# fbreitwieser/krakenuniq

Measured on AMD Instinct MI355X. Metric: Mreads/s (150 bp), higher is better.
Workload: dtype u64

## Files before the change

### krakenuniq_amd/csrc/ku_short.hip

```cpp
#include <cstdlib>
#include <type_traits>

#include "ku_device.h"

#define KS_WAVES 4
#ifndef KS_KCT_LOG2
#define KS_KCT_LOG2 8
#endif
#define KS_FLOOR_EVERY 64u
#define KS_HQ 64
#define KS_PAD 16
#ifdef KU_ABLATION
#define KS_ABL(bit) ((ablate & (bit)) != 0)
#else
#define KS_ABL(bit) false
#endif

template <int ITEMS> struct KsGeom {
  static constexpr int MAXN = 64 * ITEMS;
  static constexpr int NWORDS = (MAXN + 31 + 15) / 16 + 3;
  static constexpr int NCODES = (MAXN + 64) / 16 + 4;
  static constexpr int NAMB = (NWORDS + 1) / 2 + 2;
  static constexpr int NMM = MAXN + 64 + 32;
  static constexpr int TCAP_LOG2 = ITEMS <= 2 ? 8 : (ITEMS <= 4 ? 9 : 10);
  static constexpr int KCT_LOG2 = KS_KCT_LOG2;
  static constexpr int RCT_LOG2 = 6;
};

template <int ITEMS, bool WIN, bool SCAN, bool HQ> struct KsWaveLds {
  using G = KsGeom<ITEMS>;
  static constexpr int TCAP = 1 << G::TCAP_LOG2;
  std::conditional_t<HQ, uint2, uint32_t> hq[HQ ? KS_HQ : 0];
  uint32_t codes[SCAN ? G::NCODES : 0];
  uint32_t amb[SCAN ? G::NAMB : 0];
  uint32_t mm[SCAN ? G::NMM : 0];
  uint32_t tkey[TCAP];
  uint32_t tcnt[TCAP];
  uint32_t kk[SCAN ? 1 << G::KCT_LOG2 : 0], kc[SCAN ? 1 << G::KCT_LOG2 : 0];
  uint32_t rk[1 << G::RCT_LOG2], rc[1 << G::RCT_LOG2];
  uint32_t misc[4];
  uint16_t tlist[WIN ? TCAP : G::MAXN];
};

struct __attribute__((packed, aligned(4))) KsQuad {
  uint32_t x, y, z, w;
};
__device__ __forceinline__ uint64_t ks_quad_key(const KsQuad &q) { return ((uint64_t)q.y << 32) | q.x; }
__device__ __forceinline__ uint4 ks_quad_header(const KsQuad &q) { return make_uint4(q.x, q.y, q.z, q.w); }

__device__ __forceinline__ bool ks_less64(uint64_t a, uint64_t b) { return (int64_t)(a - b) < 0; }

__device__ __forceinline__ void ks_wave_sync() {
  __builtin_amdgcn_fence(__ATOMIC_RELEASE, "wavefront");
  __builtin_amdgcn_wave_barrier();
  __builtin_amdgcn_fence(__ATOMIC_ACQUIRE, "wavefront");
}

template <int LOG2>
__device__ __forceinline__ void ks_ct_flush(uint32_t *key, uint32_t *cnt, uint32_t *used, unsigned long long *global,
                                            uint32_t lane, uint32_t *hot = nullptr) {
  ks_wave_sync();
  for (uint32_t i = lane; i < (1u << LOG2); i += 64) {
    uint32_t kk = key[i];
#ifdef KS_DIAG_NOHOT
    if (kk == 1) kk = 0;
#endif
    if (hot && kk == 1) { *hot = cnt[i]; kk = 0; }
    if (kk) atomicAdd(&global[kk - 1], (unsigned long long)cnt[i]);
    key[i] = 0;
    cnt[i] = 0;
  }
  if (lane == 0) *used = 0;
  ks_wave_sync();
}

__device__ __forceinline__ uint32_t ks_bmin4(uint32_t a, uint32_t b) {
  const uint32_t m = ((((a | 0x80808080u) - b) & 0x80808080u) >> 7) * 0xFFu;
  return (b & m) | (a & ~m);
}

#define KS_RCT_SLOT 0x40000000u
__device__ __forceinline__ uint32_t ks_rct_node(uint32_t id, const KuTaxDev &tax) {
  return (id & KS_RCT_SLOT) ? ((id & ~KS_RCT_SLOT) ? tax.slot_node[id & ~KS_RCT_SLOT] : 0u) : id;
}
template <int LOG2>
__device__ __forceinline__ void ks_rct_add(uint32_t *key, uint32_t *cnt, uint32_t *used, uint32_t id, const KuTaxDev &tax,
                                           unsigned long long *global) {
  uint32_t h = (id * 2654435761u) >> (32 - LOG2);
#pragma unroll 1
  for (int probe = 0; probe < 8; ++probe) {
    uint32_t cur = key[h];
    if (cur == 0) { key[h] = id + 1; *used += 1; cur = id + 1; }
    if (cur == id + 1) { cnt[h] += 1; return; }
    h = (h + 1) & ((1u << LOG2) - 1);
  }
  atomicAdd(&global[ks_rct_node(id, tax)], 1ull);
}
template <int LOG2>
__device__ __forceinline__ void ks_rct_flush(uint32_t *key, uint32_t *cnt, uint32_t *used, const KuTaxDev &tax,
                                             unsigned long long *global, uint32_t lane, uint32_t *hot = nullptr) {
  ks_wave_sync();
  for (uint32_t i = lane; i < (1u << LOG2); i += 64) {
    uint32_t kk = key[i];
#ifdef KS_DIAG_NOHOT
    if (kk - 1 == KS_RCT_SLOT) kk = 0;
#endif
    if (hot && kk - 1 == KS_RCT_SLOT) { *hot = cnt[i]; kk = 0; }
    if (kk) atomicAdd(&global[ks_rct_node(kk - 1, tax)], (unsigned long long)cnt[i]);
    key[i] = 0;
    cnt[i] = 0;
  }
  if (lane == 0) *used = 0;
  ks_wave_sync();
}

template <int LOG2, bool TRACK>
__device__ __forceinline__ void ks_tab_add(uint32_t *t_key, uint32_t *t_cnt, uint32_t *n_distinct, uint32_t slot, uint32_t count) {
  uint32_t h = (slot * 2654435761u) >> (32 - LOG2);
  for (;;) {
    uint32_t cur = __hip_atomic_load(&t_key[h], __ATOMIC_RELAXED, __HIP_MEMORY_SCOPE_WORKGROUP);
    if (cur == 0) {
      uint32_t old = atomicCAS(&t_key[h], 0u, slot + 1);
      if (TRACK && old == 0) atomicAdd(n_distinct, 1u);
      cur = old == 0 ? slot + 1 : old;
    }
    if (cur == slot + 1) {
      atomicAdd(&t_cnt[h], count);
      break;
    }
    h = (h + 1) & ((1u << LOG2) - 1);
  }
}

template <int LOG2>
__device__ __forceinline__ uint32_t ks_tab_resolve(uint32_t *t_key, uint32_t *t_cnt, uint16_t *t_list, uint32_t *list_len,
                                                   const KuTaxDev &tax, uint32_t lane, uint32_t *urow = nullptr) {
  constexpr uint32_t TCAP = 1u << LOG2;
  if (lane == 0) *list_len = 0;
  ks_wave_sync();
  for (uint32_t i = lane; i < TCAP; i += 64)
    if (t_key[i]) t_list[atomicAdd(list_len, 1u)] = (uint16_t)i;
  ks_wave_sync();
  const uint32_t n_list = *list_len;
  uint32_t my_max = 0;
  for (uint32_t e = lane; e < n_list; e += 64) {
    const uint32_t pos = t_list[e];
    const uint32_t sl = t_key[pos] - 1;
    if (urow) atomicAdd(&urow[sl], t_cnt[pos] & 0xffffu);
    uint32_t score = 0;
    for (uint32_t i = tax.slot_anc_off[sl], i_end = tax.slot_anc_off[sl + 1]; i < i_end; ++i) {
      const uint32_t s = tax.slot_anc[i];
      uint32_t h = (s * 2654435761u) >> (32 - LOG2);
      for (;;) {
        const uint32_t cur = t_key[h];
        if (cur == s + 1) { score += t_cnt[h] & 0xffffu; break; }
        if (cur == 0) break;
        h = (h + 1) & (TCAP - 1);
      }
    }
    atomicAdd(&t_cnt[pos], score << 16);
    my_max = max(my_max, score);
  }
  my_max = ku_wave_max_u32(my_max);
  ks_wave_sync();
  uint32_t last = 0, res = 0;
  bool firstt = true;
  for (;;) {
    uint32_t my_min = 0xFFFFFFFFu;
    for (uint32_t e = lane; e < n_list; e += 64) {
      const uint32_t pos = t_list[e];
      const uint32_t s = t_key[pos] - 1;
      if ((t_cnt[pos] >> 16) == my_max && s > last) my_min = min(my_min, s);
    }
    my_min = ku_wave_min_u32(my_min);
    if (my_min == 0xFFFFFFFFu) break;
    const uint32_t node = tax.slot_node[my_min];
    res = firstt ? node : ku_lca_nodes(tax.node_parent, res, node);
    firstt = false;
    last = my_min;
  }
  ks_wave_sync();
  for (uint32_t e = lane; e < n_list; e += 64) {
    const uint32_t pos = t_list[e];
    t_key[pos] = 0;
    t_cnt[pos] = 0;
  }
  ks_wave_sync();
  return res;
}

__device__ __forceinline__ uint32_t ks_gload(const uint32_t *p) {
  return __hip_atomic_load(p, __ATOMIC_RELAXED, __HIP_MEMORY_SCOPE_AGENT);
}
__device__ __noinline__ void ks_floor_scan(const uint8_t *registers, uint32_t *hll_floor, uint32_t rs, uint32_t lane) {
  const uint4 *row = reinterpret_cast<const uint4 *>(registers + (size_t)rs * KU_HLL_M) + 4 * lane;
  const uint32_t cur = ks_gload(&hll_floor[rs]);
  uint32_t lo = 0x7f7f7f7fu;
#pragma unroll
  for (int q = 0; q < 4; ++q) {
    const uint4 x = row[q];
    lo = ks_bmin4(lo, ks_bmin4(ks_bmin4(x.x, x.y), ks_bmin4(x.z, x.w)));
  }
  lo = min(min(lo & 0xffu, (lo >> 8) & 0xffu), min((lo >> 16) & 0xffu, lo >> 24));
  lo = ku_wave_min_u32(lo);
  if (lane == 0 && lo > cur) atomicMax(&hll_floor[rs], lo);
}

__device__ __noinline__ void ks_hq_drain(const uint2 *q, uint32_t fill, uint8_t *registers, uint32_t lane) {
  ks_wave_sync();
  if (lane < fill) {
    const uint2 e = q[lane];
    uint8_t *r = registers + (size_t)e.x * KU_HLL_M + (e.y & (KU_HLL_M - 1u));
    ku_hll_raise(r, (uint32_t)*r, e.y >> KU_HLL_P);
  }
  ks_wave_sync();
}

__device__ __noinline__ void ks_spill_add(uint32_t *g_key, uint32_t *g_cnt, uint32_t mask, uint32_t slot, uint32_t count) {
  uint32_t h = (slot * 2654435761u) & mask;
  for (;;) {
    uint32_t cur = ks_gload(&g_key[h]);
    if (cur == 0) {
      uint32_t old = atomicCAS(&g_key[h], 0u, slot + 1);
      cur = old == 0 ? slot + 1 : old;
    }
    if (cur == slot + 1) {
      atomicAdd(&g_cnt[h], count);
      break;
    }
    h = (h + 1) & mask;
  }
}
__device__ __noinline__ void ks_spill_migrate(uint32_t *t_key, uint32_t *t_cnt, uint32_t tcap, uint32_t *g_key, uint32_t *g_cnt,
                                              uint32_t mask, bool wipe, uint32_t lane) {
  if (wipe) {
    for (uint32_t i = lane; i <= mask; i += 64) { g_key[i] = 0; g_cnt[i] = 0; }
    __threadfence();
  }
  ks_wave_sync();
  for (uint32_t i = lane; i < tcap; i += 64) {
    const uint32_t kk = t_key[i];
    if (kk) {
      ks_spill_add(g_key, g_cnt, mask, kk - 1, t_cnt[i] & 0xffffu);
      t_key[i] = 0;
      t_cnt[i] = 0;
    }
  }
  ks_wave_sync();
}
__device__ __noinline__ uint32_t ks_spill_resolve(uint32_t *g_key, uint32_t *g_cnt, uint32_t mask, const uint32_t *slot_anc_off,
                                                  const uint32_t *slot_anc, const uint32_t *slot_node, const uint32_t *node_parent,
                                                  uint32_t lane) {
  __threadfence();
  uint32_t my_max = 0;
  for (uint32_t pos = lane; pos <= mask; pos += 64) {
    const uint32_t kk = ks_gload(&g_key[pos]);
    if (!kk) continue;
    uint32_t score = 0;
    for (uint32_t i = slot_anc_off[kk - 1], i_end = slot_anc_off[kk]; i < i_end; ++i) {
      const uint32_t s = slot_anc[i];
      uint32_t h = (s * 2654435761u) & mask;
      for (;;) {
        const uint32_t cur = ks_gload(&g_key[h]);
        if (cur == s + 1) { score += ks_gload(&g_cnt[h]) & 0xffffu; break; }
        if (cur == 0) break;
        h = (h + 1) & mask;
      }
    }
    atomicAdd(&g_cnt[pos], score << 16);
    my_max = max(my_max, score);
  }
  my_max = ku_wave_max_u32(my_max);
  __threadfence();
  uint32_t last = 0, res = 0;
  bool firstt = true;
  for (;;) {
    uint32_t my_min = 0xFFFFFFFFu;
    for (uint32_t pos = lane; pos <= mask; pos += 64) {
      const uint32_t kk = ks_gload(&g_key[pos]);
      if (kk && (ks_gload(&g_cnt[pos]) >> 16) == my_max && kk - 1 > last) my_min = min(my_min, kk - 1);
    }
    my_min = ku_wave_min_u32(my_min);
    if (my_min == 0xFFFFFFFFu) break;
    const uint32_t node = slot_node[my_min];
    res = firstt ? node : ku_lca_nodes(node_parent, res, node);
    firstt = false;
    last = my_min;
  }
  for (uint32_t pos = lane; pos <= mask; pos += 64)
    if (ks_gload(&g_key[pos])) { g_key[pos] = 0; g_cnt[pos] = 0; }
  __threadfence();
  return res;
}

template <int ITEMS>
__device__ __forceinline__ uint32_t ks_g_insert_items(unsigned long long *g_key, uint64_t g_mask, const uint32_t (&slot)[ITEMS],
                                                      const uint64_t (&hash)[ITEMS], const bool (&want)[ITEMS], uint32_t *err) {
  unsigned long long key[ITEMS], old[ITEMS];
  uint64_t h[ITEMS];
#pragma unroll
  for (int j = 0; j < ITEMS; ++j) {
    key[j] = ((unsigned long long)(slot[j] + 1) << 32) | ks_encode(hash[j]);
    h[j] = ks_mix(key[j]) & g_mask;
  }
#pragma unroll
  for (int j = 0; j < ITEMS; ++j) old[j] = want[j] ? atomicCAS(&g_key[h[j]], 0ull, key[j]) : key[j];
  uint32_t fresh_n = 0;
#pragma unroll
  for (int j = 0; j < ITEMS; ++j) {
    bool fresh = want[j] && old[j] == 0ull;
    if (want[j] && old[j] != 0ull && old[j] != key[j]) {
      bool placed = false;
      for (uint32_t probe = 1; probe < 4096 && !placed; ++probe) {
        h[j] = (h[j] + 1) & g_mask;
        const unsigned long long o = atomicCAS(&g_key[h[j]], 0ull, key[j]);
        fresh = o == 0ull;
        placed = o == 0ull || o == key[j];
      }
      if (!placed) atomicOr(err, 4u);
    }
    fresh_n += (uint32_t)__popcll(__ballot(fresh));
  }
  return fresh_n;
}

#ifndef KS_OCC2
#define KS_OCC2 6
#endif
#define KS_OCC(ITEMS) ((ITEMS) == 2 ? KS_OCC2 : 4)
template <int ITEMS, bool DO_COUNTS, int KK, int MM, bool WIN, int OUT, bool ROUTE = false>
__global__ __launch_bounds__(64 * KS_WAVES, KS_OCC(ITEMS)) void ku_classify_short_kernel(
    KuDbDev db, KuTaxDev tax, KuCountsDev cnt, const uint8_t *__restrict__ seqs, uint64_t n_bytes,
    const uint64_t *__restrict__ seq_off, const uint32_t *__restrict__ seq_len, uint64_t n_reads,
    uint32_t *__restrict__ calls, uint32_t *__restrict__ taxa, uint32_t ablate, uint32_t floor_every,
    uint32_t *__restrict__ spill, uint32_t spill_cap, KuRunsOut ro, KuSparseFast sf, KuRouteIn rin) {
  using G = KsGeom<ITEMS>;
  constexpr uint32_t TCAP = 1u << G::TCAP_LOG2;
  using Lds = KsWaveLds<ITEMS, WIN, !ROUTE, DO_COUNTS && !ROUTE>;
  __shared__ Lds s_w[KS_WAVES];

  const uint32_t lane = threadIdx.x & 63u;
  const uint32_t wv = (uint32_t)__builtin_amdgcn_readfirstlane((int)(threadIdx.x >> 6));
  Lds &sw = s_w[wv];
  uint32_t *codes = sw.codes, *amb = sw.amb, *mmv = sw.mm;
  uint32_t *t_key = sw.tkey, *t_cnt = sw.tcnt;
  uint16_t *t_list = sw.tlist;
  uint16_t *amb16 = reinterpret_cast<uint16_t *>(amb);
  uint32_t *misc = sw.misc;
  const uint32_t k = KK ? (uint32_t)KK : db.k, m = KK ? (uint32_t)MM : db.nt, w = k - m + 1;
  const uint32_t key_shift = ku_key_shift(m);
  const uint32_t *tab = reinterpret_cast<const uint32_t *>(db.table);

  for (uint32_t i = lane; i < TCAP; i += 64) { t_key[i] = 0; t_cnt[i] = 0; }
  if (!ROUTE)
    for (uint32_t i = lane; i < (1u << G::KCT_LOG2); i += 64) { sw.kk[i] = 0; sw.kc[i] = 0; }
  for (uint32_t i = lane; i < (1u << G::RCT_LOG2); i += 64) { sw.rk[i] = 0; sw.rc[i] = 0; }
  if (lane < 4) misc[lane] = 0;
  ks_wave_sync();

  const uint32_t n_waves = gridDim.x * KS_WAVES;
  uint32_t *g_key = WIN ? spill + ((uint64_t)blockIdx.x * KS_WAVES + wv) * 2ull * spill_cap : nullptr;
  uint32_t *g_cnt = WIN ? g_key + spill_cap : nullptr;
  bool spill_used = false;
  unsigned long long ch_pos = 0, ch_end = 0;
  if (OUT != 0 && ro.pre_base1) {
    ch_pos = ((unsigned long long)(ro.pre_base1 - 1u) + (unsigned long long)blockIdx.x * KS_WAVES + wv) * ro.chunk;
    ch_end = ch_pos + ro.chunk;
  }
  auto runs_room = [&](uint32_t need, uint32_t keep, unsigned long long &keep_base) {
    if (ch_pos + need <= ch_end) return;
    const uint32_t want_min = keep ? 2u * (keep + need) : need;
    const uint32_t want = want_min > ro.chunk ? want_min : ro.chunk;
    unsigned long long b = 0;
    if (lane == 0) b = atomicAdd(ro.counter, (unsigned long long)want);
    b = ((unsigned long long)(uint32_t)__builtin_amdgcn_readfirstlane((int)(uint32_t)(b >> 32)) << 32) |
        (uint32_t)__builtin_amdgcn_readfirstlane((int)(uint32_t)b);
    if (keep) {
      __threadfence();
      for (uint32_t i = lane; i < keep; i += 64) {
        if (keep_base + i < ro.cap && b + i < ro.cap) {
          const uint32_t *src = reinterpret_cast<const uint32_t *>(ro.runs + keep_base + i);
          ro.runs[b + i] = make_uint2(ks_gload(src), ks_gload(src + 1));
        }
      }
      keep_base = b;
    }
    ch_pos = b + keep;
    ch_end = b + want;
  };
  uint32_t sp_fresh = 0;
  uint32_t fl_reads =
      floor_every ? (((uint32_t)blockIdx.x * KS_WAVES + wv) * 40503u >> 8) % floor_every : 0u;
  uint32_t fl_scan = 0;
  uint32_t hq_fill = 0;
  uint2 *hq = reinterpret_cast<uint2 *>(sw.hq);
  uint32_t len_n = 0;
  uint64_t off_n = 0;
  {
    const uint64_t r0 = (uint64_t)blockIdx.x * KS_WAVES + wv;
    if (ks_less64(r0, n_reads)) { len_n = seq_len[r0]; off_n = seq_off[r0]; }
  }
  for (uint64_t r = (uint64_t)blockIdx.x * KS_WAVES + wv; ks_less64(r, n_reads); r += n_waves) {
    const uint32_t rlen = len_n;
    const uint64_t roff = off_n;
    {
      const uint64_t rn = r + n_waves;
      const bool more = ks_less64(rn, n_reads);
      len_n = more ? seq_len[rn] : 0u;
      off_n = more ? seq_off[rn] : 0ull;
    }
    const uint32_t n_all = rlen >= k ? rlen - k + 1 : 0;
    uint32_t rd_first = 0, rd_cnt = 0, win0 = 0;
    bool rd_table = false, rd_spill = false;
    uint32_t call_node = 0;
    unsigned long long run_base = 0;
    uint32_t run_n = 0, run_prev = 0;
    bool run_has_prev = false;
    do {
    const uint32_t len = WIN ? min(rlen - win0, (uint32_t)G::MAXN + k - 1) : rlen;
    const uint64_t off = roff + win0;
    const uint32_t n = len >= k ? len - k + 1 : 0;
    if (DO_COUNTS) {
      if (!ROUTE && fl_scan) {
        ks_floor_scan(cnt.registers, cnt.hll_floor, fl_scan - 1u, lane);
        fl_scan = 0;
      }
      const uint32_t fill_k = misc[0], fill_r = misc[1];
      if (!ROUTE && fill_k > (1u << G::KCT_LOG2) / 2) ks_ct_flush<G::KCT_LOG2>(sw.kk, sw.kc, &misc[0], cnt.n_kmers, lane);
      if (!WIN || win0 == 0)
        if (fill_r > (1u << G::RCT_LOG2) / 2) ks_rct_flush<G::RCT_LOG2>(sw.rk, sw.rc, &misc[1], tax, cnt.n_reads, lane);
    }
    uint32_t v[ITEMS];
    bool amb_k[ITEMS];
    uint64_t hh[ITEMS];
#pragma unroll
    for (int j = 0; j < ITEMS; ++j) { v[j] = 0; amb_k[j] = false; hh[j] = 0; }

    if (ROUTE) {
      uint32_t tk[ITEMS], kbv[ITEMS];
#pragma unroll
      for (int j = 0; j < ITEMS; ++j) {
        const uint32_t p = j * 64 + lane;
        tk[j] = p < n ? taxa[off + p] : KU_ROUTE_MISS;
      }
#pragma unroll
      for (int j = 0; j < ITEMS; ++j) {
        amb_k[j] = tk[j] == KU_AMBIG;
        kbv[j] = tk[j] < KU_ROUTE_MISS ? rin.kb[tk[j] >> 5] : 0u;
      }
#pragma unroll
      for (int j = 0; j < ITEMS; ++j) v[j] = tk[j] < KU_ROUTE_MISS ? rin.ret[(uint64_t)kbv[j] + (tk[j] & 31u)] : 0u;
    } else if (n > 0) {
      constexpr uint32_t S1_LANES = (uint32_t)((G::NWORDS * 4 + 63) / 64) * 64;
      constexpr bool S1_CLAMP = S1_LANES / 4 > (uint32_t)G::NCODES || S1_LANES / 4 > 2u * G::NAMB;
      static_assert(G::NCODES - 1 >= G::NWORDS && 2 * G::NAMB - 1 >= G::NWORDS + 1, "no dump element behind the code words");
      const bool text_inside = ks_less64(off + len + 6, n_bytes);
      const uint32_t *text = reinterpret_cast<const uint32_t *>(seqs + (off & ~3ull));
      const uint32_t text_sh = (uint32_t)off & 3u, last_dw = (len - 1u) & ~3u;
#pragma unroll
      for (uint32_t pl = lane; pl < S1_LANES; pl += 64) {
        const uint32_t b0 = 4 * pl;
        const uint32_t valid = len - min(b0, len);
        uint32_t c8 = 0, a4 = 0xFu;
        if (text_inside) {
          const uint32_t *q = text + (min(b0, last_dw) >> 2);
          ku_pack_dword(__builtin_amdgcn_alignbyte(q[1], q[0], text_sh), c8, a4);
        } else if (b0 < len) {
          const uint64_t a = off + b0;
          uint32_t d = 0;
          for (uint32_t j = 0; j < 4; ++j) d |= (a + j < n_bytes ? (uint32_t)seqs[a + j] : (uint32_t)'N') << (8 * j);
          ku_pack_dword(d, c8, a4);
        }
        if (valid < 4) a4 |= (1u << (4 - valid)) - 1u;
        const uint32_t q4 = pl & 3u;
        uint32_t word = c8 << (24 - 8 * q4), ab = a4 << (12 - 4 * q4);
        word |= ku_quad_xor1(word);
        ab |= ku_quad_xor1(ab);
        word |= ku_quad_xor2(word);
        ab |= ku_quad_xor2(ab);
        const uint32_t wi = pl >> 2;
        codes[S1_CLAMP ? min(wi, (uint32_t)G::NCODES - 1u) : wi] = word;
        amb16[(S1_CLAMP ? min(wi, 2u * G::NAMB - 1u) : wi) ^ 1u] = (uint16_t)ab;
      }
      ks_wave_sync();

      const uint32_t P = n + w - 1;
      uint64_t canon[ITEMS];
      bool is_fwd[ITEMS], ok[ITEMS];
      uint32_t pk[ITEMS + 1], wr[ITEMS + 1];
      uint32_t tacc = 0xFFFFFFFFu;
      bool tie = false;
      static_assert(G::MAXN + 30 + 63 < G::NMM - 1, "the sentinels reach the dump slot");
      mmv[P + lane] = (0x03FFFFFFu - lane) << KU_PK_KEYSHIFT;
      const bool tail_round = P > (uint32_t)ITEMS * 64u;
      pk[ITEMS] = 0;
      wr[ITEMS] = (uint32_t)G::NMM - 1u;
#pragma unroll
      for (int j = 0; j <= ITEMS; ++j) {
        if (j == ITEMS && !tail_round) break;
        const uint32_t p = j * 64 + lane;
        wr[j] = p < P ? p : (uint32_t)G::NMM - 1u;
        const uint32_t wi = p >> 4, sh = (p & 15u) * 2;
        const uint32_t c0 = codes[wi], c1 = codes[wi + 1], c2 = codes[wi + 2];
        const uint64_t x = ((((uint64_t)c0 << 32) | c1) << sh >> 32 << 32) | ((((uint64_t)c1 << 32) | c2) << sh >> 32);
        const uint32_t mm = (uint32_t)(x >> (64 - 2 * m));
        const uint32_t mrc = ku_revcomp32(mm, m);
        pk[j] = ku_pk_make((mm < mrc ? mm : mrc) ^ db.xor_mask, key_shift, mm <= mrc);
        if ((m & 1u) == 0) tie |= p < P && mm == mrc;
        mmv[wr[j]] = pk[j];
        if (j < ITEMS) {
          const uint64_t fwd = x >> (64 - 2 * k);
          const uint64_t rc = ku_revcomp64(fwd, k);
          is_fwd[j] = fwd <= rc;
          canon[j] = is_fwd[j] ? fwd : rc;
          const uint32_t ai = p >> 5, as = p & 31u;
          const uint32_t a = __funnelshift_l(amb[ai + 1], amb[ai], as);
          amb_k[j] = p < n && (a >> (32 - k)) != 0;
          ok[j] = p < n && !amb_k[j];
        }
      }
      ks_wave_sync();

      uint32_t key[ITEMS], aoff[ITEMS];
      bool plus[ITEMS];
      if (KS_ABL(64u)) {
#pragma unroll
        for (int j = 0; j < ITEMS; ++j) { key[j] = 0; aoff[j] = 0; plus[j] = true; }
      } else {
        uint32_t blk = 1;
        uint32_t tj[ITEMS + 1];
#pragma unroll
        for (int j = 0; j <= ITEMS; ++j) tj[j] = 0xFFFFFFFFu;
        auto doubling = [&](auto nr_c) {
          constexpr int NR = decltype(nr_c)::value;
#pragma unroll
          for (uint32_t sft = 0; sft < 5; ++sft) {
            const uint32_t st = 1u << sft;
            if (2 * st > w) break;
            uint32_t nb[NR];
#pragma unroll
            for (int j = 0; j < NR; ++j) nb[j] = mmv[j * 64 + lane + st] + (st << 1);
            ks_wave_sync();
#pragma unroll
            for (int j = 0; j < NR; ++j) {
              tj[j] = min(tj[j], (pk[j] ^ nb[j]) - 2u);
              pk[j] = min(pk[j], nb[j]);
              mmv[wr[j]] = pk[j];
            }
            ks_wave_sync();
            blk = 2 * st;
          }
        };
        if (tail_round) doubling(std::integral_constant<int, ITEMS + 1>{});
        else doubling(std::integral_constant<int, ITEMS>{});
        if (w > blk) {
#pragma unroll
          for (int j = 0; j < ITEMS; ++j) {
            const uint32_t nbj = mmv[j * 64 + lane + (w - blk)] + ((w - blk) << 1);
            tj[j] = min(tj[j], (pk[j] ^ nbj) - 2u);
            pk[j] = min(pk[j], nbj);
          }
        }
#pragma unroll
        for (int j = 0; j <= ITEMS; ++j) tacc = min(tacc, j * 64 + lane < P ? tj[j] : 0xFFFFFFFFu);
        tie |= tacc < (1u << KU_PK_KEYSHIFT) - 2u;
#pragma unroll
        for (int j = 0; j < ITEMS; ++j) {
          const uint32_t t = (pk[j] >> 1) & 31u;
          key[j] = pk[j] >> KU_PK_KEYSHIFT;
          aoff[j] = is_fwd[j] ? t : w - 1 - t;
          plus[j] = ((pk[j] & 1u) != 0) == is_fwd[j];
        }
        if (__any(tie)) {
          ks_wave_sync();
#pragma unroll
          for (int j = 0; j <= ITEMS; ++j) {
            const uint32_t p = j * 64 + lane;
            if (p < P) {
              const uint32_t wi = p >> 4, sh = (p & 15u) * 2;
              const uint64_t two = ((uint64_t)codes[wi] << 32) | codes[wi + 1];
              const uint32_t mm = (uint32_t)((two << sh) >> (64 - 2 * m));
              const uint32_t mrc = ku_revcomp32(mm, m);
              mmv[p] = (mm < mrc ? mm : mrc) ^ db.xor_mask;
            }
          }
          ks_wave_sync();
#pragma unroll
          for (int j = 0; j < ITEMS; ++j) {
            const uint32_t p = j * 64 + lane;
            if (ok[j]) {
              uint32_t bin;
              key[j] = ku_anchor_exact(mmv + p, w, key_shift, is_fwd[j], aoff[j], bin);
              const uint32_t q = p + (is_fwd[j] ? aoff[j] : w - 1 - aoff[j]);
              const uint32_t wi = q >> 4, sh = (q & 15u) * 2;
              const uint64_t two = ((uint64_t)codes[wi] << 32) | codes[wi + 1];
              const uint32_t mmf = (uint32_t)((two << sh) >> (64 - 2 * m));
              const uint32_t rcm = ku_revcomp32(mmf, m);
              plus[j] = is_fwd[j] ? (mmf <= rcm) : (rcm <= mmf);
            }
          }
        }
      }
      const uint32_t *lp[ITEMS];
      uint32_t cand[ITEMS];
      bool act[ITEMS], ovf[ITEMS];
#pragma unroll
      for (int j = 0; j < ITEMS; ++j) {
        const uint64_t locus = ku_locus_assemble(canon[j], key[j], aoff[j], plus[j], k, m);
        hh[j] = ku_fmix64(canon[j]);
        const uint64_t line = ku_locus_line(locus, db.n_lines);
        lp[j] = tab + (ok[j] ? line : 0) * KU_LINE_DWORDS;
        act[j] = ok[j] && !KS_ABL(1u);
        if (KS_ABL(64u)) lp[j] = tab;
      }

      uint4 h4[ITEMS];
#pragma unroll
      for (int j = 0; j < ITEMS; ++j) h4[j] = *reinterpret_cast<const uint4 *>(lp[j]);
      KsQuad q[ITEMS];
      const uint32_t *ep[ITEMS];
      bool nxt[ITEMS];
      const uint32_t *const tab_end = tab + db.n_lines * KU_LINE_DWORDS;
#pragma unroll
      for (int j = 0; j < ITEMS; ++j) {
        cand[j] = ku_tag_matches(h4[j], ku_table_tag(hh[j])) & (act[j] ? 0xFFu : 0u);
        ovf[j] = act[j] && ku_line_spilled(h4[j]);
        nxt[j] = ovf[j] && cand[j] == 0;
        const uint32_t eo = nxt[j] ? (uint32_t)KU_LINE_DWORDS : KU_LINE_ENTRY0 + 3 * (__builtin_ctz(cand[j] | 0x100u) & 7u);
        ep[j] = lp[j] + eo;
        if (ep[j] == tab_end) ep[j] = tab;
      }
#pragma unroll
      for (int j = 0; j < ITEMS; ++j) q[j] = *reinterpret_cast<const KsQuad *>(ep[j]);
      uint32_t sb[ITEMS];
      if (OUT == 2 && DO_COUNTS) {
#pragma unroll
        for (int j = 0; j < ITEMS; ++j)
          sb[j] = reinterpret_cast<const uint8_t *>(lp[j] + KU_LINE_SEEN0)[__builtin_ctz(cand[j] | 0x100u) & 7u];
      }
#pragma unroll
      for (int j = 0; j < ITEMS; ++j) {
        const bool hit = cand[j] != 0 && ks_quad_key(q[j]) == canon[j];
        v[j] = hit ? q[j].z : 0u;
        if (OUT == 2 && DO_COUNTS) {
          if (hit && !sb[j] && !KS_ABL(128u)) ku_seen_mark(lp[j], (uint32_t)__builtin_ctz(cand[j]));
        }
        cand[j] &= cand[j] - 1;
        act[j] = !hit && (cand[j] != 0 || ovf[j]);
      }
      bool any = false;
#pragma unroll
      for (int j = 0; j < ITEMS; ++j) any |= act[j];
      while (any && !KS_ABL(1024u)) {
        bool pick[ITEMS], taken = false, fresh = false, ov = false;
        const uint32_t *l = tab;
        uint32_t cm = 0;
        uint64_t hsel = 0;
        KsQuad hq = {0, 0, 0, 0};
#pragma unroll
        for (int j = 0; j < ITEMS; ++j) {
          pick[j] = act[j] && !taken;
          taken |= act[j];
          if (pick[j]) { hsel = hh[j]; l = lp[j]; cm = cand[j]; ov = ovf[j]; fresh = nxt[j]; hq = q[j]; }
        }
        const uint32_t t = ku_table_tag(hsel);
        if (fresh) {
          l += KU_LINE_DWORDS;
          if (l == tab_end) l = tab;
        }
        for (;;) {
          if (fresh) {
            cm = ku_tag_matches(ks_quad_header(hq), t);
            ov = ku_line_spilled(ks_quad_header(hq));
          }
          if (cm == 0 && !ov) break;
          fresh = cm == 0;
          if (fresh) {
            l += KU_LINE_DWORDS;
            if (l == tab_end) l = tab;
          }
          const uint32_t ei = (uint32_t)__builtin_ctz(cm | 0x100u) & 7u;
          hq = *reinterpret_cast<const KsQuad *>(fresh ? l : l + KU_LINE_ENTRY0 + 3 * ei);
          if (!fresh) {
            cm &= cm - 1;
            bool same = false;
#pragma unroll
            for (int j = 0; j < ITEMS; ++j) same |= pick[j] && ks_quad_key(hq) == canon[j];
            if (same) {
#pragma unroll
              for (int j = 0; j < ITEMS; ++j)
                if (pick[j]) v[j] = hq.z;
              if (OUT == 2 && DO_COUNTS && !KS_ABL(128u)) ku_seen_mark(l, ei);
              break;
            }
          }
        }
        any = false;
#pragma unroll
        for (int j = 0; j < ITEMS; ++j) {
          if (pick[j]) act[j] = false;
          any |= act[j];
        }
      }

    }

    bool uni = false;
    uint32_t uni_slot = 0;
    uint32_t hit_first = 0;
    if (!KS_ABL(32u)) {
      uint32_t mine = 0;
#pragma unroll
      for (int j = 0; j < ITEMS; ++j)
        if (mine == 0) mine = v[j];
      const unsigned long long bal = __ballot(mine != 0);
      const uint32_t first = bal ? ku_wave_bcast(mine, (uint32_t)__ffsll((long long)bal) - 1) : 0u;
      bool diff = false;
#pragma unroll
      for (int j = 0; j < ITEMS; ++j) diff |= (v[j] != 0 && v[j] != first);
      uni = !__any(diff);
      uni_slot = uni ? first : 0u;
      hit_first = first;
      if (!WIN) {
        if (!uni) {
#pragma unroll
          for (int j = 0; j < ITEMS; ++j)
            if (v[j] != 0) ks_tab_add<G::TCAP_LOG2, false>(t_key, t_cnt, nullptr, v[j], 1u);
          uint32_t *urow_hits = nullptr;
          if (OUT == 2 && DO_COUNTS && !KS_ABL(512u)) urow_hits = sf.u_cnt + (size_t)(sf.unit_of[r] - sf.unit_base) * sf.n_slots;
          call_node = ks_tab_resolve<G::TCAP_LOG2>(t_key, t_cnt, t_list, &misc[2], tax, lane, urow_hits);
        }
      } else if (bal) {
        uint32_t w_hits = 0;
#pragma unroll
        for (int j = 0; j < ITEMS; ++j) w_hits += (uint32_t)__popcll(__ballot(v[j] != 0));
        if (!rd_table && !(uni && (rd_first == 0 || rd_first == first))) {
          if (rd_first && lane == 0) ks_tab_add<G::TCAP_LOG2, true>(t_key, t_cnt, &misc[3], rd_first, rd_cnt);
          rd_table = true;
        }
        if (!rd_table) {
          rd_first = first;
          rd_cnt += w_hits;
        } else {
          ks_wave_sync();
          if (!rd_spill && misc[3] > TCAP - (uint32_t)G::MAXN - 32u) {
            ks_spill_migrate(t_key, t_cnt, TCAP, g_key, g_cnt, spill_cap - 1, !spill_used, lane);
            spill_used = true;
            rd_spill = true;
          }
          if (!rd_spill) {
            if (uni) {
              if (lane == 0) ks_tab_add<G::TCAP_LOG2, true>(t_key, t_cnt, &misc[3], first, w_hits);
            } else {
#pragma unroll
              for (int j = 0; j < ITEMS; ++j)
                if (v[j] != 0) ks_tab_add<G::TCAP_LOG2, true>(t_key, t_cnt, &misc[3], v[j], 1u);
            }
          } else {
            if (uni) {
              if (lane == 0) ks_spill_add(g_key, g_cnt, spill_cap - 1, first, w_hits);
            } else {
#pragma unroll
              for (int j = 0; j < ITEMS; ++j)
                if (v[j] != 0) ks_spill_add(g_key, g_cnt, spill_cap - 1, v[j], 1u);
            }
          }
        }
      }
    }

    const uint32_t uni_code = uni && uni_slot ? tax.slot_taxid[uni_slot] : 0u;
    const bool fl_on = DO_COUNTS && !ROUTE && floor_every != 0 && n > 0;
    uint32_t fl_miss = 0, fl_hit = 0;
    if (fl_on && uni) {
      fl_miss = ks_gload(&cnt.hll_floor[0]);
      fl_hit = ks_gload(&cnt.hll_floor[uni_slot]);
    }

    uint32_t n_hit = 0, n_miss = 0;
    if (DO_COUNTS && !ROUTE && n > 0) {
      uint32_t rank[ITEMS], fl[ITEMS];
      if (fl_on && !uni) {
#pragma unroll
        for (int j = 0; j < ITEMS; ++j) fl[j] = ks_gload(&cnt.hll_floor[v[j]]);
      } else {
#pragma unroll
        for (int j = 0; j < ITEMS; ++j) fl[j] = v[j] ? fl_hit : fl_miss;
      }
      bool go[ITEMS];
      unsigned long long gob[ITEMS];
      uint32_t n_go = 0;
#pragma unroll
      for (int j = 0; j < ITEMS; ++j) {
        const bool okc = j * 64 + lane < n && !amb_k[j];
        (void)ku_hll_locate(cnt.registers, 0u, hh[j], rank[j]);
        go[j] = okc && rank[j] > fl[j] && !KS_ABL(2u);
        gob[j] = __ballot(go[j]);
        n_go += (uint32_t)__popcll(gob[j]);
      }
      const bool direct = !fl_on || n_go > KS_HQ / 2;
      if (direct) {
        uint8_t *reg[ITEMS];
        uint32_t seen[ITEMS];
#pragma unroll
        for (int j = 0; j < ITEMS; ++j) {
          reg[j] = ku_hll_locate(cnt.registers, go[j] ? v[j] : 0u, hh[j], rank[j]);
          seen[j] = go[j] ? (uint32_t)*reg[j] : 0xFFu;
        }
#pragma unroll
        for (int j = 0; j < ITEMS; ++j) ku_hll_raise(reg[j], seen[j], rank[j]);
      } else {
        if (hq_fill + n_go > KS_HQ) {
          ks_hq_drain(hq, hq_fill, cnt.registers, lane);
          hq_fill = 0;
        }
#pragma unroll
        for (int j = 0; j < ITEMS; ++j) {
          const uint32_t at = hq_fill + __builtin_amdgcn_mbcnt_hi((uint32_t)(gob[j] >> 32), __builtin_amdgcn_mbcnt_lo((uint32_t)gob[j], 0u));
          if (go[j]) hq[at] = make_uint2(v[j], (uint32_t)(hh[j] >> (64 - KU_HLL_P)) | (rank[j] << KU_HLL_P));
          hq_fill += (uint32_t)__popcll(gob[j]);
        }
      }
#pragma unroll
      for (int j = 0; j < ITEMS; ++j) {
        const bool okc = j * 64 + lane < n && !amb_k[j];
        if (uni) {
          n_hit += (uint32_t)__popcll(__ballot(okc && v[j] != 0));
          n_miss += (uint32_t)__popcll(__ballot(okc && v[j] == 0));
        } else if (okc && !KS_ABL(4u)) {
          ku_ct_add<G::KCT_LOG2>(sw.kk, sw.kc, &misc[0], v[j], 1, cnt.n_kmers);
        }
      }
      if (uni && lane == 0 && !KS_ABL(4u)) {
        if (n_hit) ku_ct_add<G::KCT_LOG2>(sw.kk, sw.kc, &misc[0], uni_slot, n_hit, cnt.n_kmers);
        if (n_miss) ku_ct_add<G::KCT_LOG2>(sw.kk, sw.kc, &misc[0], 0u, n_miss, cnt.n_kmers);
      }
      if (fl_on && ((++fl_reads) & 0x7fffffffu) >= floor_every) {
        fl_reads = ~fl_reads & 0x80000000u;
        fl_scan = ((fl_reads >> 31) ? hit_first : 0u) + 1u;
      }
    }

    if (OUT == 2 && DO_COUNTS && n > 0) {
      uint32_t *urow = sf.u_cnt + (size_t)(sf.unit_of[r] - sf.unit_base) * sf.n_slots;
      bool any_miss;
      if (KS_ABL(512u)) {
        any_miss = false;
      } else if (uni) {
        if (lane == 0) {
          if (n_hit) atomicAdd(&urow[uni_slot], n_hit);
          if (n_miss) atomicAdd(&urow[0], n_miss);
        }
        any_miss = n_miss != 0;
      } else if (!WIN && !KS_ABL(32u)) {
        uint32_t nm = 0;
#pragma unroll
        for (int j = 0; j < ITEMS; ++j) nm += (uint32_t)__popcll(__ballot(j * 64 + lane < n && !amb_k[j] && v[j] == 0));
        if (lane == 0 && nm) atomicAdd(&urow[0], nm);
        any_miss = nm != 0;
      } else {
        unsigned long long miss_any = 0;
#pragma unroll
        for (int j = 0; j < ITEMS; ++j) {
          const bool okc = j * 64 + lane < n && !amb_k[j];
          unsigned long long todo = __ballot(okc);
          while (todo) {
            const uint32_t lead = (uint32_t)__ffsll((long long)todo) - 1u;
            const uint32_t s0 = ku_wave_bcast(v[j], lead);
            const unsigned long long same = __ballot(okc && v[j] == s0);
            if (lane == lead) atomicAdd(&urow[s0], (uint32_t)__popcll(same));
            todo &= ~same;
          }
          miss_any |= __ballot(okc && v[j] == 0);
        }
        any_miss = miss_any != 0;
      }
      if (any_miss && sf.dense[0] == 0 && !KS_ABL(256u)) {
        bool want[ITEMS];
#pragma unroll
        for (int j = 0; j < ITEMS; ++j) want[j] = j * 64 + lane < n && !amb_k[j] && v[j] == 0;
        sp_fresh += ks_g_insert_items<ITEMS>(sf.g_key, sf.g_mask, v, hh, want, sf.err);
      }
    }

    uint32_t tcode[ITEMS];
    if (uni) {
#pragma unroll
      for (int j = 0; j < ITEMS; ++j) tcode[j] = v[j] ? uni_code : 0u;
    } else {
#pragma unroll
      for (int j = 0; j < ITEMS; ++j) tcode[j] = tax.slot_taxid[v[j]];
    }
    if (OUT == 0) {
#pragma unroll
      for (int j = 0; j < ITEMS; ++j) {
        const uint32_t p = j * 64 + lane;
        if (p < n && !KS_ABL(8u)) taxa[off + p] = amb_k[j] ? KU_AMBIG : tcode[j];
      }
    } else {
      unsigned long long sm[ITEMS];
      uint32_t carry = run_prev, w_runs = 0;
#pragma unroll
      for (int j = 0; j < ITEMS; ++j) {
        tcode[j] = amb_k[j] ? KU_AMBIG : tcode[j];
        uint32_t up = ku_wave_up1(tcode[j]);
        if (lane == 0) up = carry;
        const bool first = j == 0 && lane == 0 && !run_has_prev;
        sm[j] = __ballot(j * 64 + lane < n && (tcode[j] != up || first));
        w_runs += (uint32_t)__popcll(sm[j]);
        carry = (uint32_t)__builtin_amdgcn_readlane((int)tcode[j], 63);
      }
      if (!WIN || run_n == 0) {
        unsigned long long none = 0;
        runs_room(w_runs, 0u, none);
        run_base = ch_pos;
      } else {
        runs_room(w_runs, run_n, run_base);
      }
      uint32_t before = 0;
#pragma unroll
      for (int j = 0; j < ITEMS; ++j) {
        const unsigned long long at = ch_pos + before + (uint32_t)__popcll(sm[j] & ((1ull << lane) - 1ull));
        if (((sm[j] >> lane) & 1ull) && at < ro.cap) ro.runs[at] = make_uint2(tcode[j], win0 + j * 64 + lane);
        before += (uint32_t)__popcll(sm[j]);
      }
      ch_pos += w_runs;
      run_n += w_runs;
      run_prev = carry;
      run_has_prev = true;
    }
    if (!WIN) {
      if (OUT != 0 && lane == 0) {
        ro.run_off[r] = run_base;
        ro.run_cnt[r] = run_n;
      }
      if (lane == 0) {
        calls[r] = uni ? uni_code : tax.node_taxid[call_node];
        if (DO_COUNTS) ks_rct_add<G::RCT_LOG2>(sw.rk, sw.rc, &misc[1], uni ? (KS_RCT_SLOT | uni_slot) : call_node, tax, cnt.n_reads);
      }
      ks_wave_sync();
      break;
    }
    uint32_t nxt = win0 + (uint32_t)G::MAXN;
    if (!ROUTE && nxt < n_all) {
      uint32_t last1 = 0;
      if (lane < (uint32_t)G::NAMB) {
        const uint32_t lo = 32u * lane;
        uint32_t wd = lo < len ? amb[lane] : 0u;
        if (len - lo < 32u && lo < len) wd &= ~0u << (32u - (len - lo));
        if (wd) last1 = lo + 32u - (uint32_t)__builtin_ctz(wd);
      }
      last1 = ku_wave_max_u32(last1);
      if (last1 > (uint32_t)G::MAXN) {
        const uint32_t skip_to = min(win0 + last1, n_all);
        if (OUT == 0) {
          if (nxt + lane < skip_to) taxa[roff + nxt + lane] = KU_AMBIG;
        } else if (skip_to > nxt && run_prev != KU_AMBIG) {
          runs_room(1u, run_n, run_base);
          if (lane == 0 && ch_pos < ro.cap) ro.runs[ch_pos] = make_uint2(KU_AMBIG, nxt);
          ch_pos += 1;
          run_n += 1;
          run_prev = KU_AMBIG;
        }
        nxt = skip_to;
      }
    }
    ks_wave_sync();
    win0 = nxt;
    } while (win0 < n_all);
    if (WIN) {
      uint32_t code;
      if (!rd_table) code = rd_first ? tax.slot_taxid[rd_first] : 0u;
      else {
        call_node = rd_spill ? ks_spill_resolve(g_key, g_cnt, spill_cap - 1, tax.slot_anc_off, tax.slot_anc, tax.slot_node, tax.node_parent, lane)
                             : ks_tab_resolve<G::TCAP_LOG2>(t_key, t_cnt, t_list, &misc[2], tax, lane);
        if (lane == 0) misc[3] = 0;
        code = tax.node_taxid[call_node];
      }
      if (lane == 0) {
        calls[r] = code;
        if (OUT != 0) {
          ro.run_off[r] = run_base;
          ro.run_cnt[r] = run_n;
        }
        if (DO_COUNTS) ks_rct_add<G::RCT_LOG2>(sw.rk, sw.rc, &misc[1], rd_table ? call_node : (KS_RCT_SLOT | rd_first), tax, cnt.n_reads);
      }
      ks_wave_sync();
    }
  }
#ifndef KS_DIAG_NOFLUSH
  if (DO_COUNTS) {
    ks_wave_sync();
    if (lane < 2) misc[2 + lane] = 0;
    if (!ROUTE && hq_fill) ks_hq_drain(hq, hq_fill, cnt.registers, lane);
    if (!ROUTE && fl_scan) ks_floor_scan(cnt.registers, cnt.hll_floor, fl_scan - 1u, lane);
    if (!ROUTE) ks_ct_flush<G::KCT_LOG2>(sw.kk, sw.kc, &misc[0], cnt.n_kmers, lane, &misc[2]);
    ks_rct_flush<G::RCT_LOG2>(sw.rk, sw.rc, &misc[1], tax, cnt.n_reads, lane, &misc[3]);
    __syncthreads();
    if (wv == 0 && lane < 2) {
      unsigned long long sum = 0;
#pragma unroll
      for (int q = 0; q < KS_WAVES; ++q) sum += s_w[q].misc[2 + lane];
      if (sum) atomicAdd(lane == 0 ? &cnt.n_kmers[0] : &cnt.n_reads[0], sum);
    }
  }
#endif
  if (OUT == 2 && lane == 0 && sp_fresh) atomicAdd(sf.g_count, (unsigned long long)sp_fresh);
}

static uint32_t ks_one_pass_max() { return getenv("KU_SHORT_ONE_PASS_MAX") ? (uint32_t)atoi(getenv("KU_SHORT_ONE_PASS_MAX")) : 192u; }
uint32_t ku_short_max_kmers(const KuDbDev &db) {
  const bool whole = db.bin_lo == 0 && db.bin_hi == (1ull << (2 * db.nt));
  return (db.table && whole) ? ks_one_pass_max() : 0;
}
uint32_t ku_short_max_kmers_windowed(const KuDbDev &db) {
  return ku_short_max_kmers(db) ? 65535u : 0u;
}

static unsigned ks_grid(uint64_t n_reads, int items, int n_cu) {
  const char *oe = getenv("KU_SHORT_BLOCKS_PER_CU");
  const uint64_t per_cu = oe ? (uint64_t)atoi(oe) : (n_reads < 500000 ? 1ull : 2ull) * KS_OCC(items);
  const uint64_t want = (n_reads + KS_WAVES - 1) / KS_WAVES, cap = (uint64_t)n_cu * per_cu;
  return (unsigned)(want < cap ? want : cap);
}
static uint32_t ks_spill_cap(uint32_t max_kmers, uint32_t n_slots) {
  const uint32_t distinct = max_kmers < n_slots ? max_kmers : n_slots;
  uint32_t cap = 1024;
  while (cap < 2 * distinct) cap <<= 1;
  return cap;
}
uint64_t ku_short_workspace_bytes(uint32_t max_kmers, uint32_t n_slots, uint64_t n_reads, int n_cu) {
  if (max_kmers <= ks_one_pass_max()) return 0;
  return (uint64_t)ks_grid(n_reads, 2, n_cu) * KS_WAVES * 2ull * ks_spill_cap(max_kmers, n_slots) * 4ull;
}

uint64_t ku_short_grid_waves(uint64_t n_reads, uint32_t max_kmers, int n_cu) {
  const bool windowed = max_kmers > ks_one_pass_max();
  return (uint64_t)ks_grid(n_reads, max_kmers <= 128 || windowed ? 2 : 3, n_cu) * KS_WAVES;
}

int ku_launch_classify_short(const KuDbDev &db, const KuTaxDev &tax, const KuCountsDev &cnt, const uint8_t *d_seqs,
                             uint64_t n_bytes, const uint64_t *d_seq_off, const uint32_t *d_seq_len, uint64_t n_reads,
                             uint32_t max_kmers, uint32_t flags, uint32_t *d_calls, uint32_t *d_taxa, uint32_t *d_hits,
                             void *d_workspace, uint64_t workspace_bytes, int n_cu, hipStream_t stream,
                             const KuRunsOut *runs_out, const KuSparseFast *sparse) {
  if (n_reads == 0) return KU_OK;
  const bool counts = !(flags & KU_F_NO_COUNTS);
  if (flags & KU_F_KEEP_SLOTS) return KU_EINVAL;
  if (sparse && (!runs_out || !counts)) return KU_EINVAL;
  if (!runs_out && !d_taxa) return KU_EINVAL;
  if (d_hits && hipMemsetAsync(d_hits, 0, n_reads * 4, stream) != hipSuccess) return KU_EHIP;
  const char *ab = getenv("KU_ABLATE");
  const uint32_t ablate = ab ? (uint32_t)atoi(ab) : 0u;
  const char *fe = getenv("KU_HLL_FLOOR_EVERY");
  const uint32_t floor_every = fe ? (uint32_t)(atoi(fe) > 0 ? atoi(fe) : 0) : KS_FLOOR_EVERY;
  const bool windowed = max_kmers > ks_one_pass_max();
  const int items = max_kmers <= 128 || windowed ? 2 : 3;
  const dim3 grid(ks_grid(n_reads, items, n_cu)), block(64 * KS_WAVES);
  uint32_t spill_cap = 0;
  if (windowed) {
    if (max_kmers > 65535u) return KU_EINVAL;
    spill_cap = ks_spill_cap(max_kmers, tax.n_slots);
    if (!d_workspace || workspace_bytes < (uint64_t)grid.x * KS_WAVES * 2ull * spill_cap * 4ull) return KU_EINVAL;
  }
  const KuRunsOut ro = runs_out ? *runs_out : KuRunsOut{};
  const KuSparseFast sf = sparse ? *sparse : KuSparseFast{};
  const int out = sparse ? 2 : (runs_out ? 1 : 0);
#define KS_LAUNCH(I, C, K, M, W, O)                                                                                          \
  hipLaunchKernelGGL((ku_classify_short_kernel<I, C, K, M, W, O>), grid, block, 0, stream, db, tax, cnt, d_seqs, n_bytes,    \
                     d_seq_off, d_seq_len, n_reads, d_calls, d_taxa, ablate, floor_every, (uint32_t *)d_workspace, spill_cap, ro, sf,   \
                     KuRouteIn{})
  const int geo = !counts || db.k != 31 ? 0 : (db.nt == 13 ? 13 : (db.nt == 15 ? 15 : 0));
#define KS_GEO(I, W, O)                                      \
  do {                                                       \
    if (!counts) KS_LAUNCH(I, false, 0, 0, W, (O) == 2 ? 1 : (O)); \
    else if (geo == 13) KS_LAUNCH(I, true, 31, 13, W, O);    \
    else if (geo == 15) KS_LAUNCH(I, true, 31, 15, W, O);    \
    else KS_LAUNCH(I, true, 0, 0, W, O);                     \
  } while (0)
#define KS_OUT(I, W)                  \
  do {                                \
    if (out == 0) KS_GEO(I, W, 0);    \
    else if (out == 1) KS_GEO(I, W, 1); \
    else KS_GEO(I, W, 2);             \
  } while (0)
  if (windowed) KS_OUT(2, true);
  else if (max_kmers <= 128) KS_OUT(2, false);
  else KS_OUT(3, false);
#undef KS_OUT
#undef KS_GEO
#undef KS_LAUNCH
  return hipGetLastError() == hipSuccess ? KU_OK : KU_EHIP;
}

uint32_t ku_route_resolve_max_kmers() { return 65535u; }
int ku_launch_route_resolve(const KuDbDev &db, const KuTaxDev &tax, const KuCountsDev &cnt, const uint64_t *d_seq_off,
                            const uint32_t *d_seq_len, uint64_t n_reads, uint32_t max_kmers, uint32_t flags, uint32_t *d_calls,
                            uint32_t *d_taxa, uint32_t *d_hits, const uint32_t *d_kb, const uint32_t *d_ret, void *d_workspace,
                            uint64_t workspace_bytes, int n_cu, hipStream_t stream, const KuRunsOut *runs_out) {
  if (n_reads == 0) return KU_OK;
  if (!d_taxa || !d_kb || !d_seq_off || !d_seq_len || !d_calls || max_kmers > 65535u) return KU_EINVAL;
  if (flags & (KU_F_KEEP_SLOTS | KU_F_QUICK)) return KU_EINVAL;
  if (d_hits && hipMemsetAsync(d_hits, 0, n_reads * 4, stream) != hipSuccess) return KU_EHIP;
  const bool counts = !(flags & KU_F_NO_COUNTS), windowed = max_kmers > 128;
  const dim3 grid(ks_grid(n_reads, 2, n_cu)), block(64 * KS_WAVES);
  uint32_t spill_cap = 0;
  if (windowed) {
    spill_cap = ks_spill_cap(max_kmers, tax.n_slots);
    if (!d_workspace || workspace_bytes < (uint64_t)grid.x * KS_WAVES * 2ull * spill_cap * 4ull) return KU_EINVAL;
  }
  const KuRunsOut ro = runs_out ? *runs_out : KuRunsOut{};
  const KuRouteIn rin{d_kb, d_ret};
#define KS_RLAUNCH(C, W, O)                                                                                                     \
  hipLaunchKernelGGL((ku_classify_short_kernel<2, C, 0, 0, W, O, true>), grid, block, 0, stream, db, tax, cnt, (const uint8_t *)nullptr, \
                     (uint64_t)0, d_seq_off, d_seq_len, n_reads, d_calls, d_taxa, 0u, 0u, (uint32_t *)d_workspace, spill_cap, ro, \
                     KuSparseFast{}, rin)
#define KS_RSEL(W, O)                  \
  do {                                 \
    if (counts) KS_RLAUNCH(true, W, O); \
    else KS_RLAUNCH(false, W, O);      \
  } while (0)
  if (windowed) { if (runs_out) KS_RSEL(true, 1); else KS_RSEL(true, 0); }
  else { if (runs_out) KS_RSEL(false, 1); else KS_RSEL(false, 0); }
#undef KS_RSEL
#undef KS_RLAUNCH
  return hipGetLastError() == hipSuccess ? KU_OK : KU_EHIP;
}
```

Before: 603.8.

## Prefetch next read's text and hoist per-read table loads earlier

```diff
diff --git a/krakenuniq_amd/csrc/ku_short.hip b/krakenuniq_amd/csrc/ku_short.hip
--- a/krakenuniq_amd/csrc/ku_short.hip
+++ b/krakenuniq_amd/csrc/ku_short.hip
@@ -65,7 +65,7 @@
 #ifdef KS_DIAG_NOHOT
     if (kk == 1) kk = 0;
 #endif
-    if (hot && kk == 1) { *hot = cnt[i]; kk = 0; }
+    if (hot && kk == 1) { *hot += cnt[i]; kk = 0; }
     if (kk) atomicAdd(&global[kk - 1], (unsigned long long)cnt[i]);
     key[i] = 0;
     cnt[i] = 0;
@@ -105,7 +105,7 @@
 #ifdef KS_DIAG_NOHOT
     if (kk - 1 == KS_RCT_SLOT) kk = 0;
 #endif
-    if (hot && kk - 1 == KS_RCT_SLOT) { *hot = cnt[i]; kk = 0; }
+    if (hot && kk - 1 == KS_RCT_SLOT) { *hot += cnt[i]; kk = 0; }
     if (kk) atomicAdd(&global[ks_rct_node(kk - 1, tax)], (unsigned long long)cnt[i]);
     key[i] = 0;
     cnt[i] = 0;
@@ -400,6 +400,20 @@
     const uint64_t r0 = (uint64_t)blockIdx.x * KS_WAVES + wv;
     if (ks_less64(r0, n_reads)) { len_n = seq_len[r0]; off_n = seq_off[r0]; }
   }
+  constexpr uint32_t S1_LANES = ROUTE ? 0u : (uint32_t)((G::NWORDS * 4 + 63) / 64) * 64;
+  constexpr bool AHEAD = !WIN && !ROUTE && S1_LANES == 64 && OUT != 2;
+  uint32_t tx0 = 0, tx1 = 0;
+#ifdef KU_ABLATION
+  uint32_t tf0 = 0, tf1 = 0;
+#endif
+  auto text_request = [&](bool first) {
+    const bool want = len_n >= k && ks_less64(off_n + len_n + 6, n_bytes);
+    const uint32_t *tq = reinterpret_cast<const uint32_t *>(seqs + (off_n & ~3ull)) + (min(4 * lane, (len_n - 1u) & ~3u) >> 2);
+    if (!want || (KS_ABL(2048u) && !first)) tq = reinterpret_cast<const uint32_t *>(seq_off);
+    tx0 = tq[0];
+    tx1 = tq[1];
+  };
+  if (AHEAD) text_request(true);
   for (uint64_t r = (uint64_t)blockIdx.x * KS_WAVES + wv; ks_less64(r, n_reads); r += n_waves) {
     const uint32_t rlen = len_n;
     const uint64_t roff = off_n;
@@ -451,7 +465,6 @@
 #pragma unroll
       for (int j = 0; j < ITEMS; ++j) v[j] = tk[j] < KU_ROUTE_MISS ? rin.ret[(uint64_t)kbv[j] + (tk[j] & 31u)] : 0u;
     } else if (n > 0) {
-      constexpr uint32_t S1_LANES = (uint32_t)((G::NWORDS * 4 + 63) / 64) * 64;
       constexpr bool S1_CLAMP = S1_LANES / 4 > (uint32_t)G::NCODES || S1_LANES / 4 > 2u * G::NAMB;
       static_assert(G::NCODES - 1 >= G::NWORDS && 2 * G::NAMB - 1 >= G::NWORDS + 1, "no dump element behind the code words");
       const bool text_inside = ks_less64(off + len + 6, n_bytes);
@@ -463,8 +476,19 @@
         const uint32_t valid = len - min(b0, len);
         uint32_t c8 = 0, a4 = 0xFu;
         if (text_inside) {
-          const uint32_t *q = text + (min(b0, last_dw) >> 2);
-          ku_pack_dword(__builtin_amdgcn_alignbyte(q[1], q[0], text_sh), c8, a4);
+          uint32_t d0 = tx0, d1 = tx1;
+#ifdef KU_ABLATION
+          if (AHEAD && KS_ABL(2048u)) {
+            if (ks_less64(r, n_waves)) { tf0 = d0; tf1 = d1; }
+            else { d0 = tf0; d1 = tf1; }
+          }
+#endif
+          if (!AHEAD) {
+            const uint32_t *q = text + (min(b0, last_dw) >> 2);
+            d0 = q[0];
+            d1 = q[1];
+          }
+          ku_pack_dword(__builtin_amdgcn_alignbyte(d1, d0, text_sh), c8, a4);
         } else if (b0 < len) {
           const uint64_t a = off + b0;
           uint32_t d = 0;
@@ -769,20 +793,34 @@
       }
     }
 
-    const uint32_t uni_code = uni && uni_slot ? tax.slot_taxid[uni_slot] : 0u;
+    uint32_t uni_code = KS_ABL(4096u) ? uni_slot : (uni && uni_slot ? tax.slot_taxid[uni_slot] : 0u);
     const bool fl_on = DO_COUNTS && !ROUTE && floor_every != 0 && n > 0;
     uint32_t fl_miss = 0, fl_hit = 0;
-    if (fl_on && uni) {
-      fl_miss = ks_gload(&cnt.hll_floor[0]);
-      fl_hit = ks_gload(&cnt.hll_floor[uni_slot]);
-    }
+    uint32_t fl[ITEMS], tcode[ITEMS];
+    if (uni) {
+      if (fl_on && !KS_ABL(4096u)) {
+        fl_miss = ks_gload(&cnt.hll_floor[0]);
+        fl_hit = ks_gload(&cnt.hll_floor[uni_slot]);
+      }
+    } else if (AHEAD) {
+      if (fl_on) {
+#pragma unroll
+        for (int j = 0; j < ITEMS; ++j) fl[j] = ks_gload(&cnt.hll_floor[v[j]]);
+      }
+#pragma unroll
+      for (int j = 0; j < ITEMS; ++j) tcode[j] = tax.slot_taxid[v[j]];
+      uni_code = tax.node_taxid[call_node];
+    }
+    if (AHEAD) text_request(false);
 
     uint32_t n_hit = 0, n_miss = 0;
     if (DO_COUNTS && !ROUTE && n > 0) {
-      uint32_t rank[ITEMS], fl[ITEMS];
+      uint32_t rank[ITEMS];
       if (fl_on && !uni) {
-#pragma unroll
-        for (int j = 0; j < ITEMS; ++j) fl[j] = ks_gload(&cnt.hll_floor[v[j]]);
+        if (!AHEAD) {
+#pragma unroll
+          for (int j = 0; j < ITEMS; ++j) fl[j] = ks_gload(&cnt.hll_floor[v[j]]);
+        }
       } else {
 #pragma unroll
         for (int j = 0; j < ITEMS; ++j) fl[j] = v[j] ? fl_hit : fl_miss;
@@ -883,11 +921,10 @@
       }
     }
 
-    uint32_t tcode[ITEMS];
     if (uni) {
 #pragma unroll
       for (int j = 0; j < ITEMS; ++j) tcode[j] = v[j] ? uni_code : 0u;
-    } else {
+    } else if (!AHEAD) {
 #pragma unroll
       for (int j = 0; j < ITEMS; ++j) tcode[j] = tax.slot_taxid[v[j]];
     }
@@ -935,7 +972,7 @@
         ro.run_cnt[r] = run_n;
       }
       if (lane == 0) {
-        calls[r] = uni ? uni_code : tax.node_taxid[call_node];
+        calls[r] = uni || AHEAD ? uni_code : tax.node_taxid[call_node];
         if (DO_COUNTS) ks_rct_add<G::RCT_LOG2>(sw.rk, sw.rc, &misc[1], uni ? (KS_RCT_SLOT | uni_slot) : call_node, tax, cnt.n_reads);
       }
       ks_wave_sync();
```

Result: faster. 621.4, median of 6 (+2.9%).
